# HKUST-Aerial-Robotics/FIESTA

Measured on NVIDIA H100. Metric: esdf_voxel_updates_per_s, higher is better.
Workload: dtype int32+f64

## Files before the change

### fiesta_b200/csrc/fb_exact.cu

```cuda
#include <cub/cub.cuh>
#include <stdio.h>
#include <stdlib.h>
#include <algorithm>
#include <chrono>
#include "fb_common.cuh"
#include "fb_exact.h"

#define XNONE 0xffffffffu
#define XMB_NONE 0xffffffffffffffffull

__device__ __forceinline__ void x_coords(const FbGeom &g, uint32_t ii, int &x, int &y, int &z) {
  z = ii % (unsigned)g.pz; const unsigned xy = ii / (unsigned)g.pz; y = xy % (unsigned)g.gy; x = xy / (unsigned)g.gy;
}
__device__ __forceinline__ unsigned x_d2(int x, int y, int z, uint32_t c) {
  int ox, oy, oz; fb_unpack(c, ox, oy, oz); ox -= x; oy -= y; oz -= z;
  return (unsigned)(ox * ox + oy * oy + oz * oz);
}
__device__ __forceinline__ unsigned x_dist_of(int x, int y, int z, uint32_t c) { return c < 2u ? 0xffffffffu : x_d2(x, y, z, c); }

__global__ void k_x_flag_exist(const uint32_t *list, unsigned n, const double *occ, double l_occ, uint8_t *flags, int want) {
  const unsigned i = blockIdx.x * blockDim.x + threadIdx.x;
  if (i < n) flags[i] = ((occ[list[i]] > l_occ) ? 1 : 0) == want;
}
__global__ void k_x_apply_seed(FbGeom g, const uint32_t *E, unsigned n, uint32_t *cobs, unsigned long long *LS, unsigned long long t0) {
// ... 76 lines not shown
static int x_sort_pairs(FbExact *X, const unsigned long long *kin, unsigned long long *kout, const uint32_t *vin, uint32_t *vout, unsigned n, cudaStream_t s,
                        int key_bits = 64) {
  size_t bytes = 0;
  CK(cub::DeviceRadixSort::SortPairs(nullptr, bytes, kin, kout, vin, vout, (int)n, 0, key_bits, s));
  CK(X->cub_tmp.grow(bytes, s));
  CK(cub::DeviceRadixSort::SortPairs(X->cub_tmp.p, bytes, kin, kout, vin, vout, (int)n, 0, key_bits, s));
  return FIESTA_OK;
}
int fb_exact_init(FbExact *X, const FbGeom &g, int device, cudaStream_t s) {
  const size_t P = (size_t)g.ptotal;
  CK(fb_xrelax_init());
  X->relax_blocks = fb_xrelax_blocks(device);
  if (X->relax_blocks <= 0 || X->relax_blocks > FB_X_MAX_BLOCKS) { fb_set_error("exact mode init: k_x_relax does not fit on this device"); return FIESTA_ERR_CUDA; }
  CK(X->MB.alloc(P)); CK(X->LS.alloc(P)); CK(X->tkey.alloc(P));
  CK(X->touched.alloc(P));
  CK(X->SUM.alloc(P)); CK(X->SUMg.alloc(P)); CK(cudaMemsetAsync(X->SUMg, 0, P * 4, s));
  CK(X->emask.alloc(P));
  CK(X->wstamp.alloc(P)); CK(cudaMemsetAsync(X->wstamp, 0, P * 4, s));
  for (int k = 0; k < 3; ++k) { CK(X->W[k].alloc(P)); CK(X->F[k].alloc(P)); CK(cudaMemsetAsync(X->W[k], 0, P * 4, s)); }
  for (int k = 0; k < 2; ++k) CK(X->E[k].alloc(P));
  X->dense_min = 16384u;
  if (const char *e = getenv("FIESTA_X_DENSE")) { long v = atol(e); if (v >= 0 && v <= (1 << 24)) X->dense_min = (unsigned)v; }
  if (const char *e = getenv("FIESTA_X_ASYNC")) X->async = atol(e) != 0;
  X->small_max = FB_X_SMALL_DEFAULT;
  if (const char *e = getenv("FIESTA_X_SMALL")) { long v = atol(e); if (v >= 0 && v <= 65536) X->small_max = (unsigned)v; }
  CK(X->slotc.alloc(((size_t)X->small_max + 1) * 32));
  const size_t c0 = P / 8 > (1u << 20) ? P / 8 : (1u << 20);
  for (FbDevBuf<unsigned long long> *b : {&X->k1, &X->k2, &X->k1b, &X->k2b}) CK(b->grow(c0, s));
  for (FbDevBuf<uint32_t> *b : {&X->dv, &X->idx[0], &X->idx[1], &X->deps, &X->nc[0], &X->nc[1], &X->sel}) CK(b->grow(c0, s));
  CK(X->flags.grow(c0, s)); CK(X->flags2.grow(c0, s));
  CK(X->cub_tmp.grow(c0 * 16 + (64u << 20), s));
  CK(X->d_ctl.alloc(1)); CK(cudaMemsetAsync(X->d_ctl, 0, sizeof(FbXCtl), s));
  CK(X->h_ctl.alloc(1));
  CK(X->d_count.alloc(4)); CK(X->d_flag.alloc(4));
  CK(X->h_count.alloc(4));
  CK(cudaMemsetAsync(X->d_count, 0, 16, s)); CK(cudaMemsetAsync(X->d_flag, 0, 16, s));
  k_x_fill64<<<FB_SMS * 8, 256, 0, s>>>(X->MB, P, XMB_NONE);
  CK(cudaMemsetAsync(X->tkey, 0, P * 8, s));
  CK(cudaMemsetAsync(X->LS, 0, P * 8, s));
  X->tclock = 1; X->key_base = 0; X->key_epoch = 1; X->key_hi = 1ull << FB_KEY_BITS; X->gen_id = 0; X->wclock = 0; X->sclock = 0;
  CK(cudaGetLastError());
  return FIESTA_OK;
}

int fb_exact_queue_crossings(FbExact *X, const unsigned long long *ins_key, const uint32_t *ins_vox, const unsigned long long *del_key,
                             const uint32_t *del_vox, FbDevBuf<uint32_t> &ins, unsigned *n_ins, FbDevBuf<uint32_t> &del, unsigned *n_del,
// ... 115 lines not shown
    CK(fb_xrelax_launch(X, g, cobs, nE, X->deps, ndep_run, scratch, X->nc[0], X->flags2, occbits, ls_deps, xdbg ? X->d_dbg.p : nullptr, s));
    if (ndep_run) k_x_unset<<<nblk(ndep_run), 256, 0, s>>>(X->deps, ndep_run, scratch);
    CK(cudaMemcpyAsync(h, X->d_ctl, sizeof(FbXCtl), cudaMemcpyDeviceToHost, s));
    CK(cudaStreamSynchronize(s));
    *launches += 1;
    if (h->err) {
      if (h->err == 3u) {
        for (int k = 0; k < 3; ++k) CK(cudaMemsetAsync(X->W[k], 0, P * 4, s));
        CK(cudaMemsetAsync(X->wstamp, 0, P * 4, s));
        X->wclock = 0;
      }
      fb_set_error(h->err == 1u ? "exact mode: generation with more than 2^27 entries"
                   : h->err == 3u ? "exact mode: a wait of the asynchronous work queue exceeded its bound" : "exact mode: behaviour fixpoint did not converge");
      return FIESTA_ERR_CUDA;
    }
    X->gen_id = h->gen_id; X->wclock = h->wclock; X->tclock = h->tclock; X->sclock = h->sclock;
    st->generations = h->generations; st->reseed_rounds = h->reseed_rounds; st->eval_rounds = h->rounds; st->dense_rounds = h->dense_rounds;
    st->voxels_changed = h->voxels_changed; st->expansions = h->expansions;
    if (xdbg) {
      static unsigned long long hd[FB_X_DBG_WORDS];
      static double cyc_per_us = 0;
      if (cyc_per_us == 0) { int dev = 0, khz = 0; CK(cudaGetDevice(&dev)); CK(cudaDeviceGetAttribute(&khz, cudaDevAttrClockRate, dev)); cyc_per_us = khz / 1000.0; }
      CK(cudaMemcpy(hd, X->d_dbg, sizeof(hd), cudaMemcpyDeviceToHost));
      static const char *cat[19] = {"S", "round1", "rounds", "dense", "commit", "apply", "s.round1", "s.rounds", "s.commit", "s.apply", "top", "empty-barrier",
                                    "reseed.rounds", "reseed.assemble", "", "", "async", "", "refresh"};
      fprintf(stderr, "[x] reseed rounds %u; phases (us, count):", st->reseed_rounds);
      for (int c = 0; c < 19; ++c)
        if (*cat[c]) fprintf(stderr, " %s %.0f/%llu", cat[c], hd[FB_XDBG_PHASE + 2 * c] / cyc_per_us, hd[FB_XDBG_PHASE + 2 * c + 1]);
      fprintf(stderr, "\n");
      fprintf(stderr, "[x] round work (summed longest CTA work time us / summed list length):");
      for (int c : {1, 2, 3, 6, 7}) fprintf(stderr, " %s %.0f/%llu", cat[c], hd[FB_XDBG_WORK + 2 * c] / cyc_per_us, hd[FB_XDBG_WORK + 2 * c + 1]);
      fprintf(stderr, "\n");
      for (int h = 0; h < 2; ++h) {
        fprintf(stderr, "[x] list-length histogram %s (log2 bucket=rounds):", h ? "s.rounds" : "rounds");
        for (int b = 0; b < 32; ++b) if (hd[FB_XDBG_NWH + 32 * h + b]) fprintf(stderr, " %d=%llu", b, hd[FB_XDBG_NWH + 32 * h + b]);
        fprintf(stderr, "\n");
      }
      fprintf(stderr, "[x] async: evaluations %llu dirty %llu pushes %llu spin %.0f us\n", hd[FB_XDBG_Q + 0], hd[FB_XDBG_Q + 1], hd[FB_XDBG_Q + 2],
              hd[FB_XDBG_Q + 3] / cyc_per_us);
      for (int gq = 0; gq < 2; ++gq) { fprintf(stderr, "[x] gen %d work lists:", gq); for (int r = 0; r < 512 && hd[FB_XDBG_ROUNDS + gq * 512 + r]; ++r) fprintf(stderr, " %llu", hd[FB_XDBG_ROUNDS + gq * 512 + r]); fprintf(stderr, "\n"); }
      fprintf(stderr, "[x] work-list entries: evaluated %llu refreshed %llu reseeded %llu\n", hd[FB_XDBG_PHASE + 2 * 14], hd[FB_XDBG_PHASE + 2 * 14 + 1], hd[FB_XDBG_PHASE + 2 * 15]);
      fprintf(stderr, "[x] gens %u rounds %u dense %u deps %u nE0 %u |", st->generations, st->eval_rounds, st->dense_rounds, st->dependants, nE);
      for (unsigned q = 0; q < st->generations && q < FB_XDBG_GENS; ++q) fprintf(stderr, " %llu/%llu/%.1fus", hd[3 * q], hd[3 * q + 1], hd[3 * q + 2] / cyc_per_us);
      fprintf(stderr, "\n");
    }
  }
  X->scratch_clean = scratch_ok;
  return FIESTA_OK;
}
```

### fiesta_b200/csrc/fb_exact.h

```cpp
#pragma once
#include "fb_common.cuh"

#define FB_X_MAX_BLOCKS 256
#define FB_X_SMALL_DEFAULT 32768u
#define FB_XDBG_GENS 1024
#define FB_XDBG_NCAT 24
#define FB_XDBG_NQ 8
#define FB_XDBG_PHASE (3 * FB_XDBG_GENS)
#define FB_XDBG_ROUNDS (FB_XDBG_PHASE + 2 * FB_XDBG_NCAT)
#define FB_XDBG_WMAX (FB_XDBG_ROUNDS + 2 * 512)
#define FB_XDBG_WORK (FB_XDBG_WMAX + 4096)
#define FB_XDBG_NWH (FB_XDBG_WORK + 2 * FB_XDBG_NCAT)
#define FB_XDBG_Q (FB_XDBG_NWH + 2 * 32)
#define FB_X_DBG_WORDS (FB_XDBG_Q + FB_XDBG_NQ)

struct FbExactStats {
  unsigned long long expansions;
  unsigned long long voxels_changed;
  unsigned generations, eval_rounds, dense_rounds, reseed_rounds, dependants;
};

struct FbXCtl {
  unsigned bar, err;
  unsigned sclock, pad1;
// ... 9 lines not shown

struct FbExact {
  FbDevBuf<unsigned long long> MB;
  FbDevBuf<unsigned long long> LS;
  FbDevBuf<unsigned long long> tkey;
  FbDevBuf<uint32_t> touched;
  unsigned long long tclock = 0;
  unsigned long long key_base = 0;
  unsigned long long key_hi = 0;
  unsigned key_epoch = 0;
  FbDevBuf<unsigned> d_count, d_flag;
  FbHostBuf<unsigned> h_count;
  bool scratch_clean = false;
  FbDevBuf<uint4> SUM;
  FbDevBuf<uint32_t> SUMg;
  unsigned gen_id = 0, wclock = 0, sclock = 0;
  FbDevBuf<uint32_t> emask;
  FbDevBuf<uint32_t> W[3], F[3];
  FbDevBuf<uint32_t> wstamp;
  FbDevBuf<uint32_t> slotc;
  unsigned dense_min = 0;
  unsigned small_max = 0;
  bool async = true;
  FbDevBuf<FbXCtl> d_ctl;
  FbHostBuf<FbXCtl> h_ctl;
  FbDevBuf<unsigned long long> d_dbg;
  int relax_blocks = 0;
  FbDevBuf<uint32_t> E[2], sel;
  FbDevBuf<unsigned long long> k1, k2, k1b, k2b;
  FbDevBuf<uint32_t> dv, idx[2], deps, nc[2];
  FbDevBuf<uint8_t> flags, flags2;
  FbDevBuf<char> cub_tmp;
};

int fb_exact_init(FbExact *X, const FbGeom &g, int device, cudaStream_t s);
int fb_exact_queue_crossings(FbExact *X, const unsigned long long *ins_key, const uint32_t *ins_vox, const unsigned long long *del_key,
                             const uint32_t *del_vox, FbDevBuf<uint32_t> &ins, unsigned *n_ins, FbDevBuf<uint32_t> &del, unsigned *n_del,
                             cudaStream_t s, int *launches);
int fb_exact_next_epoch(FbExact *X, const FbGeom &g, cudaStream_t s);
int fb_exact_update_esdf(FbExact *X, const FbGeom &g, uint32_t *cobs, uint32_t *scratch, const double *occ, const uint32_t *occbits, double l_occ,
                         const uint32_t *ins, unsigned n_ins, const uint32_t *del, unsigned n_del, cudaStream_t s, FbExactStats *st, int *launches);
cudaError_t fb_xrelax_init();
int fb_xrelax_blocks(int device);
cudaError_t fb_xrelax_launch(FbExact *X, const FbGeom &g, uint32_t *cobs, unsigned nE0, const uint32_t *deps, unsigned ndep, uint32_t *ord, uint32_t *nc, uint8_t *nk,
                             const uint32_t *occbits, unsigned long long ls_deps, unsigned long long *dbg, cudaStream_t s);
```

### fiesta_b200/csrc/fb_xrelax.cu

```cuda
#include <stdio.h>
#include "fb_common.cuh"
#include "fb_exact.h"
#include "fb_divmagic.h"

#define XT 1024
#define XW (XT / 32)
#define XNONE 0xffffffffu
#define X_DEAD 0ull
#define X_PULL 1ull
#define X_PUSH 2ull
#define XMB_NONE 0xffffffffffffffffull
#define X_NOFF 129
#define X_MAX_ROUNDS 4000000u
#define XGB 8
#define XRC 8
#define XDBG_PHASE FB_XDBG_PHASE
#define XDBG_ROUNDS FB_XDBG_ROUNDS
#define XDBG_WMAX FB_XDBG_WMAX

static __constant__ int x_dirs[24][3] = {
    {-1, 0, 0}, {1, 0, 0}, {0, -1, 0}, {0, 1, 0}, {0, 0, -1}, {0, 0, 1},
    {-1, -1, 0}, {1, 1, 0}, {0, -1, -1}, {0, 1, 1}, {-1, 0, -1}, {1, 0, 1},
    {-1, 1, 0}, {1, -1, 0}, {0, -1, 1}, {0, 1, -1}, {1, 0, -1}, {-1, 0, 1},
    {-2, 0, 0}, {2, 0, 0}, {0, -2, 0}, {0, 2, 0}, {0, 0, -2}, {0, 0, 2}};
// ... 127 lines not shown

struct XArgs {
  FbGeom g;
  uint32_t *cobs;
  unsigned long long *MB, *LS;
  uint4 *SUM;
  uint32_t *SUMg;
  uint32_t *E[2];
  uint32_t *emask;
  uint32_t *W[3], *F[3];
  uint32_t *wstamp;
  uint32_t *slotc;
  FbXCtl *ctl;
  unsigned nE0, small_max, dense_min;
  const uint32_t *deps; unsigned ndep;
  uint32_t *ord;
  uint32_t *nc;
  uint8_t *nk;
  const uint32_t *occbits;
  unsigned long long ls_deps;
  unsigned long long *dbg;
  unsigned div_pz_m, div_pz_s, div_gy_m, div_gy_s;
  unsigned async_on;
};
__device__ __forceinline__ unsigned x_div(unsigned n, unsigned m, unsigned s) { return m ? (__umulhi(n, m) >> s) : n; }
__device__ __forceinline__ void x_coords(const XArgs &a, uint32_t ii, int &x, int &y, int &z) {
  const unsigned xy = x_div(ii, a.div_pz_m, a.div_pz_s);
  z = (int)(ii - xy * (unsigned)a.g.pz);
  const unsigned xx = x_div(xy, a.div_gy_m, a.div_gy_s);
  y = (int)(xy - xx * (unsigned)a.g.gy);
  x = (int)xx;
}

__device__ __forceinline__ void x_unpack_off(int o, int &dx, int &dy, int &dz) { dx = (o & 15) - 4; dy = ((o >> 4) & 15) - 4; dz = ((o >> 8) & 15) - 4; }

__device__ __forceinline__ void x_claim_summaries(const XArgs &a, const XShared &sh, unsigned lane, int x, int y, int z, unsigned sclock) {
  if (lane >= 25u) return;
  int dx, dy, dz; x_unpack_off(sh.dir[lane], dx, dy, dz);
  const int nx = x + dx, ny = y + dy, nz = z + dz;
  if (!x_in_grid(a.g, nx, ny, nz) || !(lane == 24u || x_in_range(a.g, nx, ny, nz))) return;
  const unsigned n = x_vi(a.g, nx, ny, nz);
  if (__ldcg(&a.SUMg[n]) != sclock && atomicExch(&a.SUMg[n], sclock) != sclock) x_summarize(a.g, a.cobs, a.MB, a.SUM, nx, ny, nz);
}

__device__ __forceinline__ void x_refresh_summaries(const XArgs &a, const XShared &sh, unsigned lane, unsigned i, uint32_t p, int x, int y, int z) {
  unsigned long long w = 0;
// ... 218 lines not shown
  if (total == 0u) return 0u;
  const int leader = __ffs(act) - 1;
  unsigned base = 0;
  if ((int)lane == leader) base = atomicAdd(counter, total);
  return __shfl_sync(act, base, leader) + pre;
}

#define X_Q_FULL 0x80000000u
#define X_Q_WAIT_NS 2000000000ull
__device__ __forceinline__ unsigned x_ld_relaxed(const unsigned *p) {
  unsigned v;
  asm volatile("ld.relaxed.gpu.global.u32 %0, [%1];" : "=r"(v) : "l"(p) : "memory");
  return v;
}
__device__ __forceinline__ unsigned long long x_globaltimer() {
  unsigned long long t;
  asm volatile("mov.u64 %0, %%globaltimer;" : "=l"(t));
  return t;
}
__device__ __forceinline__ void x_q_abort(const XArgs &a) {
  atomicCAS(&a.ctl->err, 0u, 3u);
  atomicExch(&a.ctl->qdone, 1u);
}
__device__ __forceinline__ unsigned x_q_count(const XArgs &a, unsigned long long delta) {
  const unsigned long long old = atomicAdd(&a.ctl->qtail, delta);
  if ((unsigned)((old + delta) >> 32) == 0u) atomicExch(&a.ctl->qdone, 1u);
  return (unsigned)old;
}
__device__ __forceinline__ void x_q_put(const XArgs &a, XShared &sh, uint32_t *ring, unsigned cap, unsigned idx, unsigned e) {
  unsigned *slot = &ring[idx % cap];
  const volatile unsigned *done = &sh.qdone;
  unsigned cur = x_ld_relaxed(slot);
  const unsigned long long t0 = x_globaltimer();
  for (unsigned it = 0;; ++it) {
    if (!(cur & X_Q_FULL)) {
      const unsigned o = atomicCAS(slot, cur, e | X_Q_FULL);
      if (o == cur) return;
      cur = o;
      continue;
    }
    if (*done) return;
    if ((it & 15u) == 15u) {
      if (x_ld_acquire(&a.ctl->qdone)) { sh.qdone = 1u; return; }
      if (x_globaltimer() - t0 > X_Q_WAIT_NS) { x_q_abort(a); sh.qdone = 1u; return; }
    }
    __nanosleep(64);
    cur = x_ld_relaxed(slot);
  }
}
__device__ __forceinline__ unsigned x_q_take(const XArgs &a, XShared &sh, uint32_t *ring, unsigned cap, unsigned &h) {
  if (h == XNONE) h = atomicAdd(&a.ctl->qhead, 1u);
  unsigned *slot = &ring[h % cap];
  const volatile unsigned *done = &sh.qdone;
  const long long c0 = a.dbg ? clock64() : 0;
  unsigned long long t0 = 0;
  unsigned ns = 32;
  for (unsigned it = 0;; ++it) {
    if (x_ld_relaxed(slot) & X_Q_FULL) {
      const unsigned v = atomicExch(slot, 0u);
      if (v & X_Q_FULL) { h = XNONE; if (a.dbg) atomicAdd(&a.dbg[FB_XDBG_Q + 3], (unsigned long long)(clock64() - c0)); return v & ~X_Q_FULL; }
    }
    if (*done) break;
    if ((it & 15u) == 15u) {
      if (x_ld_acquire(&a.ctl->qdone)) { sh.qdone = 1u; break; }
      const unsigned long long t = x_globaltimer();
      if (t0 == 0) t0 = t;
      else if (t - t0 > X_Q_WAIT_NS) { x_q_abort(a); sh.qdone = 1u; break; }
    }
    __nanosleep(ns);
    ns = ns < 256u ? 2u * ns : 256u;
  }
  if (a.dbg) atomicAdd(&a.dbg[FB_XDBG_Q + 3], (unsigned long long)(clock64() - c0));
  return XNONE;
}
__device__ __forceinline__ unsigned x_q_list(const XArgs &a, XShared &sh, const XNb &nb, uint32_t *ring, unsigned cap, unsigned lane, unsigned i, unsigned nof, unsigned A) {
  unsigned j[5], st[5];
#pragma unroll
  for (int t = 0; t < 5; ++t) {
    const unsigned o = lane + 32u * (unsigned)t;
    const unsigned long long w = o < nof ? nb.w[o] : XMB_NONE;
    j[t] = w != XMB_NONE ? x_mb_idx(w) : 0u;
    st[t] = (w != XMB_NONE && j[t] > i) ? x_ld_relaxed(&a.wstamp[j[t]]) : A + 1u;
  }
  unsigned pm = 0;
#pragma unroll
  for (int t = 0; t < 5; ++t)
    if (st[t] != A + 1u && atomicMax(&a.wstamp[j[t]], A + 1u) < A) pm |= 1u << t;
  const unsigned cnt = (unsigned)__popc(pm);
  unsigned incl = cnt;
#pragma unroll
  for (int o = 1; o < 32; o <<= 1) { const unsigned v = __shfl_up_sync(0xffffffffu, incl, o); if ((int)lane >= o) incl += v; }
  const unsigned total = __shfl_sync(0xffffffffu, incl, 31);
  if (total == 0u) return 0u;
  unsigned base = 0;
  if (lane == 0) base = x_q_count(a, (unsigned long long)total * 0x100000001ull);
  base = __shfl_sync(0xffffffffu, base, 0) + incl - cnt;
#pragma unroll
  for (int t = 0; t < 5; ++t) if ((pm >> t) & 1u) x_q_put(a, sh, ring, cap, base++, j[t]);
  return total;
}
__device__ void x_async(const XArgs &a, XShared &sh, XNb &stg, unsigned lane, unsigned gwarp, unsigned gwarps, const uint32_t *E, unsigned nE,
                        const uint32_t *wl, unsigned nw, uint32_t *ring, unsigned gen, unsigned A, unsigned fout) {
  for (unsigned q0 = gwarp * 32u; q0 < nw; q0 += gwarps * 32u) {
    const unsigned q = q0 + lane;
    const unsigned e = q < nw ? __ldcg(&wl[q]) : 0u;
    const bool push = q < nw && atomicMax(&a.wstamp[e], A + 1u) < A;
    const unsigned pm = __ballot_sync(0xffffffffu, push), cnt = (unsigned)__popc(pm);
    if (cnt == 0u) continue;
    unsigned base = 0;
    if (lane == 0) base = x_q_count(a, (unsigned long long)cnt * 0x100000001ull);
    base = __shfl_sync(0xffffffffu, base, 0);
    if (push) x_q_put(a, sh, ring, nE, base + (unsigned)__popc(pm & ((1u << lane) - 1u)), e);
    if (a.dbg && lane == 0) atomicAdd(&a.dbg[FB_XDBG_Q + 2], (unsigned long long)cnt);
  }
  if (lane == 0) x_q_count(a, 0ull - (1ull << 32));
  unsigned h = XNONE;
  for (;;) {
    unsigned i = 0;
    if (lane == 0) i = x_q_take(a, sh, ring, nE, h);
    i = __shfl_sync(0xffffffffu, i, 0);
    if (i == XNONE) break;
    const uint32_t p = __ldcg(&E[i]);
    int x, y, z; x_coords(a, p, x, y, z);
    for (;;) {
      if (a.dbg && lane == 0) atomicAdd(&a.dbg[FB_XDBG_Q + 0], 1ull);
      if (lane == 0) atomicExch(&a.wstamp[i], A);
      __syncwarp();
      __threadfence();
      x_stage(a, sh, stg, lane, x, y, z);
      const unsigned long long old = stg.w[0], nw2 = x_eval_nb(a, sh, stg, lane, gen, i, x, y, z);
      if (nw2 != old) {
        if (lane == 0) {
          a.MB[p] = nw2;
          const unsigned f = atomicAdd(&a.ctl->nF[fout], 1u);
          if (f < (unsigned)a.g.ptotal) a.F[fout][f] = i;
        }
        __syncwarp();
        __threadfence();
        const unsigned np = x_q_list(a, sh, stg, ring, nE, lane, i, (x_mb_kind(old) == X_PUSH || x_mb_kind(nw2) == X_PUSH) ? (unsigned)X_NOFF : 25u, A);
        if (a.dbg && lane == 0 && np) atomicAdd(&a.dbg[FB_XDBG_Q + 2], (unsigned long long)np);
      }
      unsigned again = 0;
      if (lane == 0) again = atomicCAS(&a.wstamp[i], A, A - 1u) != A ? 1u : 0u;
      if (!__shfl_sync(0xffffffffu, again, 0)) break;
      if (a.dbg && lane == 0) atomicAdd(&a.dbg[FB_XDBG_Q + 1], 1ull);
    }
    if (lane == 0) x_q_count(a, 0ull - (1ull << 32));
  }
}

__device__ __forceinline__ uint32_t x_reseed_eval(const XArgs &a, unsigned i, int x, int y, int z, unsigned &kc) {
  const FbGeom &g = a.g;
  kc = 24u;
  for (int k = 0; k < 24; ++k) {
    const int nx = x + x_dirs[k][0], ny = y + x_dirs[k][1], nz = z + x_dirs[k][2];
    if (!x_in_range(g, nx, ny, nz) || !x_in_grid(g, nx, ny, nz)) continue;
    const unsigned nv = x_vi(g, nx, ny, nz);
    const unsigned o = __ldcg(&a.ord[nv]);
    uint32_t c;
    if (o != XNONE) { if (o < i) c = __ldcg(&a.nc[o]); else continue; }
    else c = __ldcg(&a.cobs[nv]) & FB_CODE_MASK;
    if (c >= 2u) {
      int ox, oy, oz; fb_unpack(c, ox, oy, oz);
      const unsigned oi = x_vi(g, ox, oy, oz);
      if ((__ldg(&a.occbits[oi >> 5]) >> (oi & 31)) & 1u) { kc = (unsigned)k; return c; }
    }
  }
  return FB_INF;
}

extern __shared__ __align__(16) unsigned char x_dyn_smem[];

__global__ void __launch_bounds__(XT, 1) k_x_relax(const XArgs a) {
  __shared__ XShared sh;
  const FbGeom &g = a.g;
  FbXCtl *ctl = a.ctl;
  const unsigned tid = threadIdx.x, lane = tid & 31u, wid = tid >> 5;
  const unsigned G = gridDim.x, b = blockIdx.x;
  const unsigned gtid = b * XT + tid, gthreads = G * XT;
  const unsigned gwarp = gtid >> 5, gwarps = gthreads >> 5;
  for (unsigned k = tid; k < X_NOFF; k += XT) sh.off[k] = x_off_c[k];
  if (tid < 32) sh.self[tid] = 0;
  if (tid == 0) sh.qdone = 0u;
  if (gtid == 0) a.ctl->qtail = (unsigned long long)gwarps << 32;
  if (tid < 32) sh.dir[tid] = tid < 24 ? ((x_dirs[tid][0] + 4) | ((x_dirs[tid][1] + 4) << 4) | ((x_dirs[tid][2] + 4) << 8)) : (4 | (4 << 4) | (4 << 8));
  __syncthreads();
  for (unsigned q = tid; q < 25u * 24u + 25u; q += XT) {
    const unsigned t = q < 600u ? q / 24u : q - 600u, k = q < 600u ? q % 24u : 24u;
    int tx, ty, tz, kx = 0, ky = 0, kz = 0; x_unpack_off(sh.dir[t], tx, ty, tz);
    if (k < 24u) x_unpack_off(sh.dir[k], kx, ky, kz);
    const int code = (tx - kx + 4) | ((ty - ky + 4) << 4) | ((tz - kz + 4) << 8);
    unsigned found = 0;
    for (unsigned o = 0; o < X_NOFF; ++o) if (sh.off[o] == code) found = o;
    if (q < 600u) sh.slot[q] = (unsigned char)found; else sh.self[t] = (unsigned char)found;
  }
  __syncthreads();
  XNb &stg = reinterpret_cast<XNb *>(x_dyn_smem)[wid];

  unsigned nE = a.nE0, bar_target = 0;
  int cur = 0;
  unsigned gen = ctl->gen_id, wclock = ctl->wclock;
  unsigned long long tclock = ctl->tclock;
  unsigned generations = 0, rounds_total = 0, dense_total = 0;
  unsigned long long changed_total = 0;
  if (a.dbg) {
    const long long t0 = clock64();
    for (int q = 0; q < 32; ++q) x_gsync(&ctl->bar, bar_target);
    if (gtid == 0) a.dbg[XDBG_PHASE + 2 * 11] = (unsigned long long)(clock64() - t0) / 32ull;
  }
  long long t_ph = a.dbg ? clock64() : 0;
#define X_LAP(cat) do { if (a.dbg && gtid == 0) { const long long t_now = clock64(); a.dbg[XDBG_PHASE + 2 * (cat)] += (unsigned long long)(t_now - t_ph); a.dbg[XDBG_PHASE + 2 * (cat) + 1] += 1ull; t_ph = t_now; } } while (0)
  unsigned reseed_rounds = 0;
  if (a.ndep) {
    for (unsigned r = 1;; ++r) {
      const unsigned in = r % 3u, out = (r + 1u) % 3u, zz = (r + 2u) % 3u;
      const unsigned nw = r == 1u ? a.ndep : __ldcg(&ctl->nW[in]);
      if (gtid == 0) ctl->nW[zz] = 0;
      if (r > 1u && nw == 0u) break;
      if (a.dbg && gtid == 0) a.dbg[XDBG_PHASE + 2 * 15] += nw;
      ++reseed_rounds; ++wclock;
      if (nw <= 2u * gwarps) {
        for (unsigned q = gwarp; q < nw; q += gwarps) {
          const unsigned i = r == 1u ? q : __ldcg(&a.W[in][q]);
          int x, y, z; x_coords(a, __ldcg(&a.deps[i]), x, y, z);
          int dx = 0, dy = 0, dz = 0;
          if (lane < 24u) x_unpack_off(sh.dir[lane], dx, dy, dz);
          const int nx = x + dx, ny = y + dy, nz = z + dz;
          const bool ing = lane < 24u && x_in_grid(g, nx, ny, nz);
          const unsigned nv = ing ? x_vi(g, nx, ny, nz) : 0u;
          const unsigned o = ing ? __ldcg(&a.ord[nv]) : XNONE;
          uint32_t c = 0;
          if (ing && x_in_range(g, nx, ny, nz)) {
            if (o != XNONE) { if (o < i) c = __ldcg(&a.nc[o]); }
            else c = __ldcg(&a.cobs[nv]) & FB_CODE_MASK;
          }
          bool ok = false;
          if (c >= 2u) { int px, py, pz; fb_unpack(c, px, py, pz); const unsigned oi = x_vi(g, px, py, pz); ok = (__ldg(&a.occbits[oi >> 5]) >> (oi & 31)) & 1u; }
          const unsigned vm = __ballot_sync(0xffffffffu, ok);
          const unsigned kc = vm ? (unsigned)(__ffs(vm) - 1) : 24u;
          const uint32_t res = vm ? __shfl_sync(0xffffffffu, c, (int)kc) : FB_INF;
          uint32_t was = 0;
          if (lane == 0) { was = __ldcg(&a.nc[i]); a.nk[i] = (uint8_t)kc; }
// ... 77 lines not shown
        a.cobs[v] = c;
        a.LS[v] = a.ls_deps + i;
      }
      unsigned ctot;
      const unsigned pos = x_block_scan(sh, (i < hi && c >= 2u) ? 1u : 0u, lane, wid, ctot);
      if (i < hi && c >= 2u) a.E[0][run + pos] = v;
      run += ctot;
    }
    nE += sh.total;
    x_gsync(&ctl->bar, bar_target);
    X_LAP(13);
  }
  bool big = nE > a.small_max;

  ++gen;
  unsigned sclock = ctl->sclock;
  for (unsigned i = gtid; i < nE; i += gthreads) {
    const uint32_t v = __ldcg(&a.E[0][i]);
    a.MB[v] = x_mb(gen, i, X_PUSH, __ldcg(&a.cobs[v]) & FB_CODE_MASK);
  }
  x_gsync(&ctl->bar, bar_target);

  while (nE) {
    const long long t_gen = a.dbg ? clock64() : 0;
    X_LAP(10);
    ++generations;
    const uint32_t *E = a.E[cur];
    unsigned rounds = 0;
    bool aborted = false;
    if (big) {
      ++sclock;
      for (unsigned i = gwarp; i < nE; i += gwarps) { int x, y, z; x_coords(a, __ldcg(&E[i]), x, y, z); x_claim_summaries(a, sh, lane, x, y, z, sclock); }
      x_gsync(&ctl->bar, bar_target);
      X_LAP(0);
    }
    for (unsigned r = 1;; ++r) {
      const unsigned in = r % 3u, out = (r + 1u) % 3u, zz = (r + 2u) % 3u;
      const unsigned nw = r == 1u ? nE : __ldcg(&ctl->nW[in]);
      const unsigned nf = (big && r > 1u) ? __ldcg(&ctl->nF[in]) : 0u;
      if (gtid == 0) { ctl->nW[zz] = 0; ctl->nF[zz] = 0; }
      if (r > 1u && nw == 0u && nf == 0u) break;
      if (r > X_MAX_ROUNDS) { if (gtid == 0) ctl->err = 2u; break; }
      if (a.dbg && gtid == 0) { a.dbg[XDBG_PHASE + 2 * 14] += nw; a.dbg[XDBG_PHASE + 2 * 14 + 1] += nf; }
      if (a.async_on && big && r > 1u && nw <= a.dense_min) {
        ++rounds; wclock += 3u;
        const unsigned A = wclock - 1u;
        x_async(a, sh, stg, lane, gwarp, gwarps, E, nE, a.W[in], nw, a.W[out], gen, A, out);
        x_gsync(&ctl->bar, bar_target);
        X_LAP(16);
        if (tid == 0) sh.qdone = 0u;
        if (gtid == 0) { ctl->qtail = (unsigned long long)gwarps << 32; ctl->qhead = 0u; ctl->qdone = 0u; }
        if (__ldcg(&ctl->err)) { aborted = true; break; }
        const unsigned nfa = __ldcg(&ctl->nF[out]);
        if (nfa > (unsigned)g.ptotal) {
          ++sclock;
          for (unsigned i = gwarp; i < nE; i += gwarps) { int x, y, z; x_coords(a, __ldcg(&E[i]), x, y, z); x_claim_summaries(a, sh, lane, x, y, z, sclock); }
        } else {
          for (unsigned q = gwarp; q < nf + nfa; q += gwarps) {
            const unsigned i = q < nf ? __ldcg(&a.F[in][q]) : __ldcg(&a.F[out][q - nf]);
            const uint32_t p = __ldcg(&E[i]);
            int x, y, z; x_coords(a, p, x, y, z);
            x_refresh_summaries(a, sh, lane, i, p, x, y, z);
          }
        }
        x_gsync(&ctl->bar, bar_target);
        X_LAP(18);
        break;
      }
      ++rounds; ++wclock;
      const bool dense = big && r > 1u && nw > a.dense_min;
      if (dense) {
        ++dense_total;
        if (nf < nE / 4u) {
          for (unsigned q = gwarp; q < nf; q += gwarps) {
            const unsigned i = __ldcg(&a.F[in][q]);
            const uint32_t p = __ldcg(&E[i]);
            int x, y, z; x_coords(a, p, x, y, z);
            x_refresh_summaries(a, sh, lane, i, p, x, y, z);
          }
        } else {
          ++sclock;
          for (unsigned i = gwarp; i < nE; i += gwarps) { int x, y, z; x_coords(a, __ldcg(&E[i]), x, y, z); x_claim_summaries(a, sh, lane, x, y, z, sclock); }
        }
        x_gsync(&ctl->bar, bar_target);
      }
      const bool use_sum = big && (r == 1u || dense);
      const unsigned nref = (big && !dense) ? nf : 0u;
      const uint32_t *wl = a.W[in];
      const long long t_w0 = a.dbg ? clock64() : 0;
      for (unsigned q = gwarp; q < nw + nref; q += gwarps) {
        if (q >= nw) {
          const unsigned i = __ldcg(&a.F[in][q - nw]);
          const uint32_t p = __ldcg(&E[i]);
          int x, y, z; x_coords(a, p, x, y, z);
          x_refresh_summaries(a, sh, lane, i, p, x, y, z);
          continue;
        }
        const unsigned i = r == 1u ? q : __ldcg(&wl[q]);
        const uint32_t p = __ldcg(&E[i]);
        int x, y, z; x_coords(a, p, x, y, z);
        if (!use_sum) {
          x_stage(a, sh, stg, lane, x, y, z);
          const unsigned long long old = stg.w[0], nw2 = x_eval_nb(a, sh, stg, lane, gen, i, x, y, z);
          if (nw2 == old) continue;
          if (lane == 0) {
            a.MB[p] = nw2;
            if (big) a.F[out][atomicAdd(&ctl->nF[out], 1u)] = i;
          }
          x_list_affected_nb(a, stg, lane, i, (x_mb_kind(old) == X_PUSH || x_mb_kind(nw2) == X_PUSH) ? (unsigned)X_NOFF : 25u, wclock, out);
          continue;
        }
        unsigned long long old = 0;
        if (lane == 0) old = __ldcg(&a.MB[p]);
        const unsigned long long nb = x_eval<true>(a, sh, lane, gen, i, p, x, y, z);
        old = __shfl_sync(0xffffffffu, old, 0);
        if (nb == old) continue;
        if (lane == 0) {
          a.MB[p] = nb;
          if (big) a.F[out][atomicAdd(&ctl->nF[out], 1u)] = i;
        }
        x_list_affected(a, sh, lane, i, x, y, z, (x_mb_kind(old) == X_PUSH || x_mb_kind(nb) == X_PUSH) ? (unsigned)X_NOFF : 25u, wclock, out);
      }
      if (a.dbg) { __syncthreads(); if (tid == 0) atomicMax(&a.dbg[XDBG_WMAX + ((rounds_total + rounds) & 4095u)], (unsigned long long)(clock64() - t_w0)); }
      x_gsync(&ctl->bar, bar_target);
      X_LAP(big ? (r == 1u ? 1 : (dense ? 3 : 2)) : (r == 1u ? 6 : 7));
      if (a.dbg && gtid == 0) {
        if (generations <= 2u && rounds <= 512u) a.dbg[XDBG_ROUNDS + (generations - 1u) * 512u + (rounds - 1u)] = nw;
        const unsigned cat = big ? (r == 1u ? 1u : (dense ? 3u : 2u)) : (r == 1u ? 6u : 7u);
        unsigned long long *wm = &a.dbg[XDBG_WMAX + ((rounds_total + rounds) & 4095u)];
        a.dbg[FB_XDBG_WORK + 2 * cat] += __ldcg(wm); a.dbg[FB_XDBG_WORK + 2 * cat + 1] += nw; *wm = 0;
        if (cat == 2u || cat == 7u) a.dbg[FB_XDBG_NWH + (cat == 7u ? 32u : 0u) + (nw ? 32u - __clz(nw) : 0u)] += 1ull;
      }
    }
    rounds_total += rounds;
    if (rounds > X_MAX_ROUNDS || aborted) break;

    const unsigned per = (nE + G - 1u) / G;
    const unsigned lo = min(nE, b * per), hi = min(nE, lo + per);
    unsigned wcount = 0, wlive = 0;
    for (unsigned i = lo + wid; i < hi; i += XW) {
      const uint32_t p = __ldcg(&E[i]);
      int x, y, z; x_coords(a, p, x, y, z);
      unsigned long long w = 0;
      if (!big) { x_stage(a, sh, stg, lane, x, y, z); w = stg.w[0]; }
      else { if (lane == 0) w = __ldcg(&a.MB[p]); w = __shfl_sync(0xffffffffu, w, 0); }
      const unsigned long long kind = x_mb_kind(w);
      bool win = false;
      if ((kind == X_PUSH && lane < 24) || (kind == X_PULL && lane == 24)) {
        int dx, dy, dz; x_unpack_off(sh.dir[lane], dx, dy, dz);
// ... 45 lines not shown
        if (w != XMB_NONE && x_mb_par(w) == (gen & 1u)) atomicCAS(&a.MB[p], w, XMB_NONE);
      }
      unsigned ctot;
      unsigned r = run + x_block_scan(sh, (unsigned)__popc(m), lane, wid, ctot);
      if (m) {
        const uint32_t p = __ldcg(&E[i]);
        int x, y, z; x_coords(a, p, x, y, z);
        uint32_t me = m;
        while (me) {
          const int k = __ffs(me) - 1; me &= me - 1u;
          int dx, dy, dz; x_unpack_off(sh.dir[k], dx, dy, dz);
          const uint32_t v = (uint32_t)x_vi(g, x + dx, y + dy, z + dz);
          const unsigned ts = i * 32u + (unsigned)k;
          const uint32_t code = big ? __ldcg(&a.SUM[v]).z : __ldcg(&a.slotc[ts]);
          a.cobs[v] = code;
          a.LS[v] = tclock + ts;
          En[r] = v;
          a.MB[v] = x_mb(gen + 1u, r, X_PUSH, code);
          ++r;
        }
      }
      run += ctot;
    }
    if (a.dbg && gtid == 0 && generations <= FB_XDBG_GENS) { a.dbg[3 * (generations - 1u)] = nE; a.dbg[3 * (generations - 1u) + 1] = rounds; a.dbg[3 * (generations - 1u) + 2] = (unsigned long long)(clock64() - t_gen); }
    tclock += (unsigned long long)nE * 32ull + 1ull;
    changed_total += n2;
    if (n2 >= (1u << 27)) { if (gtid == 0) ctl->err = 1u; break; }
    const bool was_big = big;
    nE = n2; cur ^= 1; big = big2; ++gen;
    x_gsync(&ctl->bar, bar_target);
    X_LAP(was_big ? 5 : 9);
  }
  if (gtid == 0) {
    ctl->gen_id = gen; ctl->wclock = wclock; ctl->tclock = tclock; ctl->sclock = sclock;
    ctl->generations = generations; ctl->reseed_rounds = reseed_rounds; ctl->rounds = rounds_total; ctl->dense_rounds = dense_total; ctl->voxels_changed = changed_total;
  }
}

static bool g_off_ready = false;
cudaError_t fb_xrelax_init() {
  if (g_off_ready) return cudaSuccess;
  static const int D[24][3] = {
      {-1, 0, 0}, {1, 0, 0}, {0, -1, 0}, {0, 1, 0}, {0, 0, -1}, {0, 0, 1},
      {-1, -1, 0}, {1, 1, 0}, {0, -1, -1}, {0, 1, 1}, {-1, 0, -1}, {1, 0, 1},
      {-1, 1, 0}, {1, -1, 0}, {0, -1, 1}, {0, 1, -1}, {1, 0, -1}, {-1, 0, 1},
      {-2, 0, 0}, {2, 0, 0}, {0, -2, 0}, {0, 2, 0}, {0, 0, -2}, {0, 0, 2}};
  int off[1024], n = 0;
  for (int p = -1; p < 24; ++p)
    for (int q = -1; q < 24; ++q) {
      int o[3];
      for (int k = 0; k < 3; ++k) o[k] = (p < 0 ? 0 : D[p][k]) + (q < 0 ? 0 : D[q][k]);
      const int code = (o[0] + 4) | ((o[1] + 4) << 4) | ((o[2] + 4) << 8);
      bool dup = false;
      for (int j = 0; j < n; ++j) dup = dup || off[j] == code;
      if (!dup) off[n++] = code;
    }
  if (n != X_NOFF) return cudaErrorUnknown;
  cudaError_t e = cudaMemcpyToSymbol(x_off_c, off, sizeof(int) * X_NOFF);
  if (e == cudaSuccess) g_off_ready = true;
  return e;
}

int fb_xrelax_blocks(int device) {
  int per_sm = 0, sms = 0;
  if (cudaOccupancyMaxActiveBlocksPerMultiprocessor(&per_sm, k_x_relax, XT, sizeof(XNb) * XW) != cudaSuccess || per_sm < 1) return -1;
  if (cudaDeviceGetAttribute(&sms, cudaDevAttrMultiProcessorCount, device) != cudaSuccess) return -1;
  return sms;
}

cudaError_t fb_xrelax_launch(FbExact *X, const FbGeom &g, uint32_t *cobs, unsigned nE0, const uint32_t *deps, unsigned ndep, uint32_t *ord, uint32_t *nc, uint8_t *nk,
                             const uint32_t *occbits, unsigned long long ls_deps, unsigned long long *dbg, cudaStream_t s) {
  XArgs a;
  a.deps = deps; a.ndep = ndep; a.ord = ord; a.nc = nc; a.nk = nk; a.occbits = occbits; a.ls_deps = ls_deps;
  fb_div_make((unsigned)g.pz, a.div_pz_m, a.div_pz_s);
  fb_div_make((unsigned)g.gy, a.div_gy_m, a.div_gy_s);
  a.g = g;
  if (a.g.max_vec[0] < a.g.min_vec[0] || a.g.max_vec[1] < a.g.min_vec[1] || a.g.max_vec[2] < a.g.min_vec[2])
    for (int k = 0; k < 3; ++k) a.g.min_vec[k] = a.g.max_vec[k] = 0x3fffffff;
  a.cobs = cobs; a.MB = X->MB; a.LS = X->LS; a.SUM = X->SUM; a.SUMg = X->SUMg;
  a.E[0] = X->E[0]; a.E[1] = X->E[1]; a.emask = X->emask;
  for (int k = 0; k < 3; ++k) { a.W[k] = X->W[k]; a.F[k] = X->F[k]; }
  a.wstamp = X->wstamp; a.slotc = X->slotc; a.ctl = X->d_ctl; a.nE0 = nE0; a.small_max = X->small_max; a.dense_min = X->dense_min; a.dbg = dbg;
  a.async_on = X->async ? 1u : 0u;
  void *args[] = {(void *)&a};
  return cudaLaunchCooperativeKernel((void *)k_x_relax, dim3(X->relax_blocks), dim3(XT), args, sizeof(XNb) * XW, s);
}
```

Baseline: 125.6 million.

## Add opt-in async work queue for small generations and template kernel on debug flag

Adds an asynchronous work-queue path for the first round of small generations, where warps claim entries by stamp and requeue affected neighbours instead of running barrier-separated rounds. It is gated behind a new environment flag that is off by default. The relax kernel is also templated on a debug flag so that timing and counter instrumentation compiles out of the normal build, and queue completion is mirrored into shared memory. The default path mainly gains from dropping runtime debug checks, at the cost of an extra kernel instantiation.

Result: faster. 129.8 million, median of 6 (+3.3%).

```diff
diff --git a/fiesta_b200/csrc/fb_exact.cu b/fiesta_b200/csrc/fb_exact.cu
--- a/fiesta_b200/csrc/fb_exact.cu
+++ b/fiesta_b200/csrc/fb_exact.cu
@@ -122,6 +122,7 @@
   X->dense_min = 16384u;
   if (const char *e = getenv("FIESTA_X_DENSE")) { long v = atol(e); if (v >= 0 && v <= (1 << 24)) X->dense_min = (unsigned)v; }
   if (const char *e = getenv("FIESTA_X_ASYNC")) X->async = atol(e) != 0;
+  if (const char *e = getenv("FIESTA_X_SMALL_ASYNC")) X->small_async = atol(e) != 0;
   X->small_max = FB_X_SMALL_DEFAULT;
   if (const char *e = getenv("FIESTA_X_SMALL")) { long v = atol(e); if (v >= 0 && v <= 65536) X->small_max = (unsigned)v; }
   CK(X->slotc.alloc(((size_t)X->small_max + 1) * 32));
@@ -283,10 +284,10 @@
       static double cyc_per_us = 0;
       if (cyc_per_us == 0) { int dev = 0, khz = 0; CK(cudaGetDevice(&dev)); CK(cudaDeviceGetAttribute(&khz, cudaDevAttrClockRate, dev)); cyc_per_us = khz / 1000.0; }
       CK(cudaMemcpy(hd, X->d_dbg, sizeof(hd), cudaMemcpyDeviceToHost));
-      static const char *cat[19] = {"S", "round1", "rounds", "dense", "commit", "apply", "s.round1", "s.rounds", "s.commit", "s.apply", "top", "empty-barrier",
-                                    "reseed.rounds", "reseed.assemble", "", "", "async", "", "refresh"};
+      static const char *cat[20] = {"S", "round1", "rounds", "dense", "commit", "apply", "s.round1", "s.rounds", "s.commit", "s.apply", "top", "empty-barrier",
+                                    "reseed.rounds", "reseed.assemble", "", "", "async", "", "refresh", "s.async"};
       fprintf(stderr, "[x] reseed rounds %u; phases (us, count):", st->reseed_rounds);
-      for (int c = 0; c < 19; ++c)
+      for (int c = 0; c < 20; ++c)
         if (*cat[c]) fprintf(stderr, " %s %.0f/%llu", cat[c], hd[FB_XDBG_PHASE + 2 * c] / cyc_per_us, hd[FB_XDBG_PHASE + 2 * c + 1]);
       fprintf(stderr, "\n");
       fprintf(stderr, "[x] round work (summed longest CTA work time us / summed list length):");
diff --git a/fiesta_b200/csrc/fb_exact.h b/fiesta_b200/csrc/fb_exact.h
--- a/fiesta_b200/csrc/fb_exact.h
+++ b/fiesta_b200/csrc/fb_exact.h
@@ -55,6 +55,7 @@
   unsigned dense_min = 0;
   unsigned small_max = 0;
   bool async = true;
+  bool small_async = false;
   FbDevBuf<FbXCtl> d_ctl;
   FbHostBuf<FbXCtl> h_ctl;
   FbDevBuf<unsigned long long> d_dbg;
diff --git a/fiesta_b200/csrc/fb_xrelax.cu b/fiesta_b200/csrc/fb_xrelax.cu
--- a/fiesta_b200/csrc/fb_xrelax.cu
+++ b/fiesta_b200/csrc/fb_xrelax.cu
@@ -173,6 +173,7 @@
   unsigned long long *dbg;
   unsigned div_pz_m, div_pz_s, div_gy_m, div_gy_s;
   unsigned async_on;
+  unsigned small_async_on;
 };
 __device__ __forceinline__ unsigned x_div(unsigned n, unsigned m, unsigned s) { return m ? (__umulhi(n, m) >> s) : n; }
 __device__ __forceinline__ void x_coords(const XArgs &a, uint32_t ii, int &x, int &y, int &z) {
@@ -437,9 +438,9 @@
   atomicCAS(&a.ctl->err, 0u, 3u);
   atomicExch(&a.ctl->qdone, 1u);
 }
-__device__ __forceinline__ unsigned x_q_count(const XArgs &a, unsigned long long delta) {
+__device__ __forceinline__ unsigned x_q_count(const XArgs &a, XShared &sh, unsigned long long delta) {
   const unsigned long long old = atomicAdd(&a.ctl->qtail, delta);
-  if ((unsigned)((old + delta) >> 32) == 0u) atomicExch(&a.ctl->qdone, 1u);
+  if ((unsigned)((old + delta) >> 32) == 0u) { atomicExch(&a.ctl->qdone, 1u); sh.qdone = 1u; }
   return (unsigned)old;
 }
 __device__ __forceinline__ void x_q_put(const XArgs &a, XShared &sh, uint32_t *ring, unsigned cap, unsigned idx, unsigned e) {
@@ -463,17 +464,18 @@
     cur = x_ld_relaxed(slot);
   }
 }
+template <bool DBG>
 __device__ __forceinline__ unsigned x_q_take(const XArgs &a, XShared &sh, uint32_t *ring, unsigned cap, unsigned &h) {
   if (h == XNONE) h = atomicAdd(&a.ctl->qhead, 1u);
   unsigned *slot = &ring[h % cap];
   const volatile unsigned *done = &sh.qdone;
-  const long long c0 = a.dbg ? clock64() : 0;
+  const long long c0 = DBG ? clock64() : 0;
   unsigned long long t0 = 0;
   unsigned ns = 32;
   for (unsigned it = 0;; ++it) {
     if (x_ld_relaxed(slot) & X_Q_FULL) {
       const unsigned v = atomicExch(slot, 0u);
-      if (v & X_Q_FULL) { h = XNONE; if (a.dbg) atomicAdd(&a.dbg[FB_XDBG_Q + 3], (unsigned long long)(clock64() - c0)); return v & ~X_Q_FULL; }
+      if (v & X_Q_FULL) { h = XNONE; if (DBG) atomicAdd(&a.dbg[FB_XDBG_Q + 3], (unsigned long long)(clock64() - c0)); return v & ~X_Q_FULL; }
     }
     if (*done) break;
     if ((it & 15u) == 15u) {
@@ -485,7 +487,7 @@
     __nanosleep(ns);
     ns = ns < 256u ? 2u * ns : 256u;
   }
-  if (a.dbg) atomicAdd(&a.dbg[FB_XDBG_Q + 3], (unsigned long long)(clock64() - c0));
+  if (DBG) atomicAdd(&a.dbg[FB_XDBG_Q + 3], (unsigned long long)(clock64() - c0));
   return XNONE;
 }
 __device__ __forceinline__ unsigned x_q_list(const XArgs &a, XShared &sh, const XNb &nb, uint32_t *ring, unsigned cap, unsigned lane, unsigned i, unsigned nof, unsigned A) {
@@ -508,12 +510,46 @@
   const unsigned total = __shfl_sync(0xffffffffu, incl, 31);
   if (total == 0u) return 0u;
   unsigned base = 0;
-  if (lane == 0) base = x_q_count(a, (unsigned long long)total * 0x100000001ull);
+  if (lane == 0) base = x_q_count(a, sh, (unsigned long long)total * 0x100000001ull);
   base = __shfl_sync(0xffffffffu, base, 0) + incl - cnt;
 #pragma unroll
   for (int t = 0; t < 5; ++t) if ((pm >> t) & 1u) x_q_put(a, sh, ring, cap, base++, j[t]);
   return total;
 }
+template <bool BIG, bool DBG>
+__device__ __forceinline__ void x_q_run(const XArgs &a, XShared &sh, XNb &stg, unsigned lane, const uint32_t *E, unsigned nE, uint32_t *ring,
+                                        unsigned gen, unsigned A, unsigned fout, unsigned i, bool claimed) {
+  const uint32_t p = __ldcg(&E[i]);
+  int x, y, z; x_coords(a, p, x, y, z);
+  for (;; claimed = false) {
+    if (DBG && lane == 0) atomicAdd(&a.dbg[FB_XDBG_Q + 0], 1ull);
+    if (!claimed) {
+      if (lane == 0) atomicExch(&a.wstamp[i], A);
+      __syncwarp();
+      __threadfence();
+    }
+    x_stage(a, sh, stg, lane, x, y, z);
+    const unsigned long long old = stg.w[0], nw2 = x_eval_nb(a, sh, stg, lane, gen, i, x, y, z);
+    if (nw2 != old) {
+      if (lane == 0) {
+        a.MB[p] = nw2;
+        if (BIG) {
+          const unsigned f = atomicAdd(&a.ctl->nF[fout], 1u);
+          if (f < (unsigned)a.g.ptotal) a.F[fout][f] = i;
+        }
+      }
+      __syncwarp();
+      __threadfence();
+      const unsigned np = x_q_list(a, sh, stg, ring, nE, lane, i, (x_mb_kind(old) == X_PUSH || x_mb_kind(nw2) == X_PUSH) ? (unsigned)X_NOFF : 25u, A);
+      if (DBG && lane == 0 && np) atomicAdd(&a.dbg[FB_XDBG_Q + 2], (unsigned long long)np);
+    }
+    unsigned again = 0;
+    if (lane == 0) again = atomicCAS(&a.wstamp[i], A, A - 1u) != A ? 1u : 0u;
+    if (!__shfl_sync(0xffffffffu, again, 0)) break;
+    if (DBG && lane == 0) atomicAdd(&a.dbg[FB_XDBG_Q + 1], 1ull);
+  }
+}
+template <bool DBG>
 __device__ void x_async(const XArgs &a, XShared &sh, XNb &stg, unsigned lane, unsigned gwarp, unsigned gwarps, const uint32_t *E, unsigned nE,
                         const uint32_t *wl, unsigned nw, uint32_t *ring, unsigned gen, unsigned A, unsigned fout) {
   for (unsigned q0 = gwarp * 32u; q0 < nw; q0 += gwarps * 32u) {
@@ -523,44 +559,47 @@
     const unsigned pm = __ballot_sync(0xffffffffu, push), cnt = (unsigned)__popc(pm);
     if (cnt == 0u) continue;
     unsigned base = 0;
-    if (lane == 0) base = x_q_count(a, (unsigned long long)cnt * 0x100000001ull);
+    if (lane == 0) base = x_q_count(a, sh, (unsigned long long)cnt * 0x100000001ull);
     base = __shfl_sync(0xffffffffu, base, 0);
     if (push) x_q_put(a, sh, ring, nE, base + (unsigned)__popc(pm & ((1u << lane) - 1u)), e);
-    if (a.dbg && lane == 0) atomicAdd(&a.dbg[FB_XDBG_Q + 2], (unsigned long long)cnt);
-  }
-  if (lane == 0) x_q_count(a, 0ull - (1ull << 32));
+    if (DBG && lane == 0) atomicAdd(&a.dbg[FB_XDBG_Q + 2], (unsigned long long)cnt);
+  }
+  if (lane == 0) x_q_count(a, sh, 0ull - (1ull << 32));
   unsigned h = XNONE;
   for (;;) {
     unsigned i = 0;
-    if (lane == 0) i = x_q_take(a, sh, ring, nE, h);
+    if (lane == 0) i = x_q_take<DBG>(a, sh, ring, nE, h);
     i = __shfl_sync(0xffffffffu, i, 0);
     if (i == XNONE) break;
-    const uint32_t p = __ldcg(&E[i]);
-    int x, y, z; x_coords(a, p, x, y, z);
-    for (;;) {
-      if (a.dbg && lane == 0) atomicAdd(&a.dbg[FB_XDBG_Q + 0], 1ull);
-      if (lane == 0) atomicExch(&a.wstamp[i], A);
-      __syncwarp();
-      __threadfence();
-      x_stage(a, sh, stg, lane, x, y, z);
-      const unsigned long long old = stg.w[0], nw2 = x_eval_nb(a, sh, stg, lane, gen, i, x, y, z);
-      if (nw2 != old) {
-        if (lane == 0) {
-          a.MB[p] = nw2;
-          const unsigned f = atomicAdd(&a.ctl->nF[fout], 1u);
-          if (f < (unsigned)a.g.ptotal) a.F[fout][f] = i;
-        }
-        __syncwarp();
-        __threadfence();
-        const unsigned np = x_q_list(a, sh, stg, ring, nE, lane, i, (x_mb_kind(old) == X_PUSH || x_mb_kind(nw2) == X_PUSH) ? (unsigned)X_NOFF : 25u, A);
-        if (a.dbg && lane == 0 && np) atomicAdd(&a.dbg[FB_XDBG_Q + 2], (unsigned long long)np);
-      }
-      unsigned again = 0;
-      if (lane == 0) again = atomicCAS(&a.wstamp[i], A, A - 1u) != A ? 1u : 0u;
-      if (!__shfl_sync(0xffffffffu, again, 0)) break;
-      if (a.dbg && lane == 0) atomicAdd(&a.dbg[FB_XDBG_Q + 1], 1ull);
-    }
-    if (lane == 0) x_q_count(a, 0ull - (1ull << 32));
+    x_q_run<true, DBG>(a, sh, stg, lane, E, nE, ring, gen, A, fout, i, false);
+    if (lane == 0) x_q_count(a, sh, 0ull - (1ull << 32));
+  }
+}
+template <bool DBG>
+__device__ void x_async_small(const XArgs &a, XShared &sh, XNb &stg, unsigned lane, unsigned gwarp, unsigned gwarps, const uint32_t *E, unsigned nE,
+                              uint32_t *ring, unsigned gen, unsigned A) {
+  const unsigned nwk = min(gwarps, nE);
+  if (gwarp >= nwk) return;
+  if (gwarp == 0u && lane == 0 && nwk < gwarps) x_q_count(a, sh, 0ull - ((unsigned long long)(gwarps - nwk) << 32));
+  for (unsigned s0 = gwarp; s0 < nE; s0 += 32u * nwk) {
+    const unsigned e = s0 + lane * nwk;
+    unsigned om = __ballot_sync(0xffffffffu, e < nE && atomicMax(&a.wstamp[e], A) < A);
+    __threadfence();
+    while (om) {
+      const unsigned i = s0 + (unsigned)(__ffs(om) - 1) * nwk;
+      om &= om - 1u;
+      x_q_run<false, DBG>(a, sh, stg, lane, E, nE, ring, gen, A, 0u, i, true);
+    }
+  }
+  if (lane == 0) x_q_count(a, sh, 0ull - (1ull << 32));
+  unsigned h = XNONE;
+  for (;;) {
+    unsigned i = 0;
+    if (lane == 0) i = x_q_take<DBG>(a, sh, ring, nE, h);
+    i = __shfl_sync(0xffffffffu, i, 0);
+    if (i == XNONE) break;
+    x_q_run<false, DBG>(a, sh, stg, lane, E, nE, ring, gen, A, 0u, i, false);
+    if (lane == 0) x_q_count(a, sh, 0ull - (1ull << 32));
   }
 }
 
@@ -586,6 +625,7 @@
 
 extern __shared__ __align__(16) unsigned char x_dyn_smem[];
 
+template <bool DBG>
 __global__ void __launch_bounds__(XT, 1) k_x_relax(const XArgs a) {
   __shared__ XShared sh;
   const FbGeom &g = a.g;
@@ -618,13 +658,13 @@
   unsigned long long tclock = ctl->tclock;
   unsigned generations = 0, rounds_total = 0, dense_total = 0;
   unsigned long long changed_total = 0;
-  if (a.dbg) {
+  if (DBG) {
     const long long t0 = clock64();
     for (int q = 0; q < 32; ++q) x_gsync(&ctl->bar, bar_target);
     if (gtid == 0) a.dbg[XDBG_PHASE + 2 * 11] = (unsigned long long)(clock64() - t0) / 32ull;
   }
-  long long t_ph = a.dbg ? clock64() : 0;
-#define X_LAP(cat) do { if (a.dbg && gtid == 0) { const long long t_now = clock64(); a.dbg[XDBG_PHASE + 2 * (cat)] += (unsigned long long)(t_now - t_ph); a.dbg[XDBG_PHASE + 2 * (cat) + 1] += 1ull; t_ph = t_now; } } while (0)
+  long long t_ph = DBG ? clock64() : 0;
+#define X_LAP(cat) do { if (DBG && gtid == 0) { const long long t_now = clock64(); a.dbg[XDBG_PHASE + 2 * (cat)] += (unsigned long long)(t_now - t_ph); a.dbg[XDBG_PHASE + 2 * (cat) + 1] += 1ull; t_ph = t_now; } } while (0)
   unsigned reseed_rounds = 0;
   if (a.ndep) {
     for (unsigned r = 1;; ++r) {
@@ -632,7 +672,7 @@
       const unsigned nw = r == 1u ? a.ndep : __ldcg(&ctl->nW[in]);
       if (gtid == 0) ctl->nW[zz] = 0;
       if (r > 1u && nw == 0u) break;
-      if (a.dbg && gtid == 0) a.dbg[XDBG_PHASE + 2 * 15] += nw;
+      if (DBG && gtid == 0) a.dbg[XDBG_PHASE + 2 * 15] += nw;
       ++reseed_rounds; ++wclock;
       if (nw <= 2u * gwarps) {
         for (unsigned q = gwarp; q < nw; q += gwarps) {
@@ -756,7 +796,7 @@
   x_gsync(&ctl->bar, bar_target);
 
   while (nE) {
-    const long long t_gen = a.dbg ? clock64() : 0;
+    const long long t_gen = DBG ? clock64() : 0;
     X_LAP(10);
     ++generations;
     const uint32_t *E = a.E[cur];
@@ -775,16 +815,18 @@
       if (gtid == 0) { ctl->nW[zz] = 0; ctl->nF[zz] = 0; }
       if (r > 1u && nw == 0u && nf == 0u) break;
       if (r > X_MAX_ROUNDS) { if (gtid == 0) ctl->err = 2u; break; }
-      if (a.dbg && gtid == 0) { a.dbg[XDBG_PHASE + 2 * 14] += nw; a.dbg[XDBG_PHASE + 2 * 14 + 1] += nf; }
-      if (a.async_on && big && r > 1u && nw <= a.dense_min) {
+      if (DBG && gtid == 0) { a.dbg[XDBG_PHASE + 2 * 14] += nw; a.dbg[XDBG_PHASE + 2 * 14 + 1] += nf; }
+      if (a.async_on && (big ? r > 1u && nw <= a.dense_min : r == 1u && a.small_async_on)) {
         ++rounds; wclock += 3u;
         const unsigned A = wclock - 1u;
-        x_async(a, sh, stg, lane, gwarp, gwarps, E, nE, a.W[in], nw, a.W[out], gen, A, out);
+        if (big) x_async<DBG>(a, sh, stg, lane, gwarp, gwarps, E, nE, a.W[in], nw, a.W[out], gen, A, out);
+        else x_async_small<DBG>(a, sh, stg, lane, gwarp, gwarps, E, nE, a.W[out], gen, A);
         x_gsync(&ctl->bar, bar_target);
-        X_LAP(16);
+        X_LAP(big ? 16 : 19);
         if (tid == 0) sh.qdone = 0u;
         if (gtid == 0) { ctl->qtail = (unsigned long long)gwarps << 32; ctl->qhead = 0u; ctl->qdone = 0u; }
         if (__ldcg(&ctl->err)) { aborted = true; break; }
+        if (!big) break;
         const unsigned nfa = __ldcg(&ctl->nF[out]);
         if (nfa > (unsigned)g.ptotal) {
           ++sclock;
@@ -821,7 +863,7 @@
       const bool use_sum = big && (r == 1u || dense);
       const unsigned nref = (big && !dense) ? nf : 0u;
       const uint32_t *wl = a.W[in];
-      const long long t_w0 = a.dbg ? clock64() : 0;
+      const long long t_w0 = DBG ? clock64() : 0;
       for (unsigned q = gwarp; q < nw + nref; q += gwarps) {
         if (q >= nw) {
           const unsigned i = __ldcg(&a.F[in][q - nw]);
@@ -855,10 +897,10 @@
         }
         x_list_affected(a, sh, lane, i, x, y, z, (x_mb_kind(old) == X_PUSH || x_mb_kind(nb) == X_PUSH) ? (unsigned)X_NOFF : 25u, wclock, out);
       }
-      if (a.dbg) { __syncthreads(); if (tid == 0) atomicMax(&a.dbg[XDBG_WMAX + ((rounds_total + rounds) & 4095u)], (unsigned long long)(clock64() - t_w0)); }
+      if (DBG) { __syncthreads(); if (tid == 0) atomicMax(&a.dbg[XDBG_WMAX + ((rounds_total + rounds) & 4095u)], (unsigned long long)(clock64() - t_w0)); }
       x_gsync(&ctl->bar, bar_target);
       X_LAP(big ? (r == 1u ? 1 : (dense ? 3 : 2)) : (r == 1u ? 6 : 7));
-      if (a.dbg && gtid == 0) {
+      if (DBG && gtid == 0) {
         if (generations <= 2u && rounds <= 512u) a.dbg[XDBG_ROUNDS + (generations - 1u) * 512u + (rounds - 1u)] = nw;
         const unsigned cat = big ? (r == 1u ? 1u : (dense ? 3u : 2u)) : (r == 1u ? 6u : 7u);
         unsigned long long *wm = &a.dbg[XDBG_WMAX + ((rounds_total + rounds) & 4095u)];
@@ -950,7 +992,7 @@
       }
       run += ctot;
     }
-    if (a.dbg && gtid == 0 && generations <= FB_XDBG_GENS) { a.dbg[3 * (generations - 1u)] = nE; a.dbg[3 * (generations - 1u) + 1] = rounds; a.dbg[3 * (generations - 1u) + 2] = (unsigned long long)(clock64() - t_gen); }
+    if (DBG && gtid == 0 && generations <= FB_XDBG_GENS) { a.dbg[3 * (generations - 1u)] = nE; a.dbg[3 * (generations - 1u) + 1] = rounds; a.dbg[3 * (generations - 1u) + 2] = (unsigned long long)(clock64() - t_gen); }
     tclock += (unsigned long long)nE * 32ull + 1ull;
     changed_total += n2;
     if (n2 >= (1u << 27)) { if (gtid == 0) ctl->err = 1u; break; }
@@ -991,7 +1033,8 @@
 
 int fb_xrelax_blocks(int device) {
   int per_sm = 0, sms = 0;
-  if (cudaOccupancyMaxActiveBlocksPerMultiprocessor(&per_sm, k_x_relax, XT, sizeof(XNb) * XW) != cudaSuccess || per_sm < 1) return -1;
+  for (const void *k : {(const void *)k_x_relax<false>, (const void *)k_x_relax<true>})
+    if (cudaOccupancyMaxActiveBlocksPerMultiprocessor(&per_sm, k, XT, sizeof(XNb) * XW) != cudaSuccess || per_sm < 1) return -1;
   if (cudaDeviceGetAttribute(&sms, cudaDevAttrMultiProcessorCount, device) != cudaSuccess) return -1;
   return sms;
 }
@@ -1010,6 +1053,7 @@
   for (int k = 0; k < 3; ++k) { a.W[k] = X->W[k]; a.F[k] = X->F[k]; }
   a.wstamp = X->wstamp; a.slotc = X->slotc; a.ctl = X->d_ctl; a.nE0 = nE0; a.small_max = X->small_max; a.dense_min = X->dense_min; a.dbg = dbg;
   a.async_on = X->async ? 1u : 0u;
+  a.small_async_on = X->small_async ? 1u : 0u;
   void *args[] = {(void *)&a};
-  return cudaLaunchCooperativeKernel((void *)k_x_relax, dim3(X->relax_blocks), dim3(XT), args, sizeof(XNb) * XW, s);
-}
+  return cudaLaunchCooperativeKernel(dbg ? (void *)k_x_relax<true> : (void *)k_x_relax<false>, dim3(X->relax_blocks), dim3(XT), args, sizeof(XNb) * XW, s);
+}
```
